# UltronAI/Depth-VO-Feat

Measured on AMD Instinct MI355X. Metric: KITTI 256x832 stereo-seq samples/sec fwd+bwd, higher is better.
Workload: dtype f32

## Files before the change

depth-vo-feat_amd/csrc/conv.hip:

```cpp
#include "dvf_common.h"
#include "conv_op.h"
#include "conv_pipe_host.h"
#include "conv_gather.h"
#include "conv_wgrad.h"
#include "wgrad_pipe.h"

namespace {

__device__ __forceinline__ float act_grad(float g, float yv, int act, float alpha, float beta) {
    if (act == DVF_ACT_RELU) return (yv > 0.f) ? g : 0.f;
    if (act == DVF_ACT_SIGMOID_AFFINE) {
        const float sg = (yv - beta) / alpha;
        return g * alpha * sg * (1.f - sg);
    }
    return g;
}

template <bool VEC>
__global__ __launch_bounds__(256) void act_bwd_kernel(const float *__restrict__ dy, const float *__restrict__ y,
                                                      float *__restrict__ dpre, float *dbias, int C, int HW, int act,
                                                      float alpha, float beta, int chunks, float *part = nullptr, int nper = 0) {
    __shared__ float red[4];
    const int plane = blockIdx.x / chunks, chunk = blockIdx.x - plane * chunks;
    const int c = plane % C;
// ... 558 lines not shown
    return chunks;
}

int64_t dvf_act_bwd_ws_floats(int N, int C, int HW) {
    if (N <= 0 || C <= 0 || HW <= 0) return DVF_ERR_INVALID_ARG;
    const int a = act_bwd_chunks(N, C, HW, true), b = bias_sum_chunks(N, C, HW);
    return (int64_t)C * N * (a > b ? a : b);
}

int dvf_act_bwd(const float *dy, const float *y, float *dpre, float *dbias, int N, int C, int HW, int act, float alpha,
                float beta, int accumulate_dbias, float *ws, int64_t ws_floats, void *stream) {
    if (!dy || (act != DVF_ACT_NONE && !y) || N <= 0 || C <= 0 || HW <= 0) return DVF_ERR_INVALID_ARG;
    if (!dpre && !dbias) return DVF_OK;
    hipStream_t st = dvf_stream(stream);
    if (dbias && !accumulate_dbias && hipMemsetAsync(dbias, 0, sizeof(float) * C, st) != hipSuccess) return DVF_ERR_LAUNCH;
    const bool vec = (HW % 4 == 0) && ((reinterpret_cast<uintptr_t>(dy) | reinterpret_cast<uintptr_t>(y) |
                                        reinterpret_cast<uintptr_t>(dpre)) % 16 == 0);
    const bool sums_only = !dpre && act == DVF_ACT_NONE;
    const int chunks = sums_only ? bias_sum_chunks(N, C, HW) : act_bwd_chunks(N, C, HW, dbias != nullptr);
    const int64_t planes = (int64_t)N * C;
    float *part = (dbias && ws && ws_floats >= dvf_act_bwd_ws_floats(N, C, HW)) ? ws : nullptr;
    if (sums_only) {
        const int per = ((vec ? HW >> 2 : HW) + chunks - 1) / chunks;
        const int threads = per <= 256 ? 64 : per <= 8192 ? 256 : 1024;
        if (vec) bias_sum_kernel<true><<<(unsigned)(planes * chunks), threads, 0, st>>>(dy, dbias, C, HW, chunks, part, N * chunks);
        else bias_sum_kernel<false><<<(unsigned)(planes * chunks), threads, 0, st>>>(dy, dbias, C, HW, chunks, part, N * chunks);
    } else if (vec) act_bwd_kernel<true><<<(unsigned)(planes * chunks), 256, 0, st>>>(dy, y, dpre, dbias, C, HW, act, alpha, beta, chunks, part, N * chunks);
    else act_bwd_kernel<false><<<(unsigned)(planes * chunks), 256, 0, st>>>(dy, y, dpre, dbias, C, HW, act, alpha, beta, chunks, part, N * chunks);
    DVF_LAUNCH_CHECK();
    if (part) {
        bias_finish_kernel<<<C, 64, 0, st>>>(part, dbias, N * chunks);
        DVF_LAUNCH_CHECK();
    }
    return DVF_OK;
}


int64_t dvf_conv2d_packed_floats(const dvf_conv_desc *d, const int *seg_channels, int nseg, int op_kind) {
    return conv_sizes(d, seg_channels, nseg, op_kind, false);
}

int64_t dvf_conv2d_ws_floats(const dvf_conv_desc *d, const int *seg_channels, int nseg, int op_kind) {
    return conv_sizes(d, seg_channels, nseg, op_kind, true);
}

int dvf_conv2d_pack(const dvf_conv_desc *d, const int *seg_channels, int nseg, int op_kind, const float *w, float *packed,
                    void *stream) {
    int rc = check_desc(d);
    if (rc) return rc;
    rc = check_segs(d, seg_channels, nseg);
    if (rc) return rc;
    if (!w || !packed) return DVF_ERR_INVALID_ARG;
    hipStream_t st = dvf_stream(stream);
    if (op_kind == 0) {
        ConvOp op;
        PipePlan pl;
        rc = make_fwd_op(d, seg_channels, nseg, op);
        if (!rc) rc = plan_pipe(op, pl);
        return rc ? rc : launch_pack(op, pl, w, packed, st);
    }
    if (op_kind != 1) return DVF_ERR_INVALID_ARG;
    return for_each_dgrad_seg(d, seg_channels, nseg, true, [&](const DgradSeg &v) -> int {
        return v.packed ? launch_pack(v.op, v.plan, w, packed + v.packed_off, st) : DVF_OK;
    });
}

int dvf_conv2d_fwd(const dvf_conv_desc *d, const float *const *in_segs, const int *seg_channels, int nseg,
                   const float *packed, const float *w, const float *bias, float *out, float *ws, int64_t ws_floats,
                   void *stream) {
    dvf_plan_reset();
    int rc = check_desc(d);
    if (rc) return rc;
    rc = check_segs(d, seg_channels, nseg);
    if (rc) return rc;
    if (!in_segs || !w || !out) return DVF_ERR_INVALID_ARG;
    for (int s = 0; s < nseg; ++s)
        if (!in_segs[s]) return DVF_ERR_INVALID_ARG;
    hipStream_t st = dvf_stream(stream);
    const ConvIO io{in_segs, bias, out, nullptr};
    ConvOp op;
    rc = make_fwd_op(d, seg_channels, nseg, op);
    if (packed && !rc) {
        PipePlan pl;
        rc = plan_pipe(op, pl);
        if (!rc) rc = run_pipe(op, pl, io, packed, ws, ws_floats, st);
        if (rc != DVF_ERR_UNSUPPORTED) return rc;
    }
    return fwd_unpacked(d, op, io, seg_channels, nseg, w, ws, ws_floats, st);
}

int dvf_conv2d_dgrad(const dvf_conv_desc *d, const float *dpre, const float *packed, const float *w, float *const *din_segs,
                     const int *seg_channels, int nseg, float *ws, int64_t ws_floats, const float *const *mask_segs,
                     void *stream) {
    dvf_plan_reset();
    int rc = check_desc(d);
    if (rc) return rc;
    rc = check_segs(d, seg_channels, nseg);
    if (rc) return rc;
    if (!dpre || !w || !din_segs) return DVF_ERR_INVALID_ARG;
    hipStream_t st = dvf_stream(stream);
    auto mask = [&](int s) -> const float * { return mask_segs ? mask_segs[s] : nullptr; };
    if (dvf_head_dgrad_applicable(d, nseg) || (dvf_head_applicable(d, nseg) && !packed))
        return din_segs[0] ? dvf_head_dgrad(d, dpre, w, din_segs[0], st, mask(0)) : DVF_OK;
    return for_each_dgrad_seg(d, seg_channels, nseg, packed != nullptr, [&](const DgradSeg &v) -> int {
        if (!din_segs[v.s]) return DVF_OK;
        const ConvIO io{&dpre, nullptr, din_segs[v.s], mask(v.s)};
        int r = v.packed ? run_pipe(v.op, v.plan, io, packed + v.packed_off, ws, ws_floats, st) : DVF_ERR_UNSUPPORTED;
        if (r == DVF_ERR_UNSUPPORTED) r = dgrad_unpacked(d, v.op, io, w, ws, ws_floats, st);
        return r;
    });
}

int dvf_conv2d_pack_jobs(const dvf_conv_desc *d, const int *seg_channels, int nseg, int op_kind, const float *w, float *packed,
                         void *jobs_host, int max_jobs, int *blocks_out, int *lds_bytes_out) {
    static_assert(sizeof(PackArgs) <= DVF_PACK_JOB_BYTES, "DVF_PACK_JOB_BYTES too small");
    int rc = check_desc(d);
    if (rc) return rc;
    rc = check_segs(d, seg_channels, nseg);
    if (rc) return rc;
    if (!w || !packed || !jobs_host || !blocks_out || max_jobs < 1) return DVF_ERR_INVALID_ARG;
    char *out = static_cast<char *>(jobs_host);
    int njobs = 0;
    auto emit = [&](const ConvOp &op, const PipePlan &pl, float *dst) {
        const PackArgs job = pack_job(op, pl, w, dst, &blocks_out[njobs]);
        memset(out + (size_t)njobs * DVF_PACK_JOB_BYTES, 0, DVF_PACK_JOB_BYTES);
        memcpy(out + (size_t)njobs * DVF_PACK_JOB_BYTES, &job, sizeof(job));
        if (lds_bytes_out && (int)pl.pack_lds > *lds_bytes_out) *lds_bytes_out = (int)pl.pack_lds;
        ++njobs;
    };
    if (op_kind == 0) {
        ConvOp op;
        PipePlan pl;
        rc = make_fwd_op(d, seg_channels, nseg, op);
        if (!rc) rc = plan_pipe(op, pl);
        if (rc) return rc;
        emit(op, pl, packed);
        return njobs;
    }
    if (op_kind != 1) return DVF_ERR_INVALID_ARG;
    rc = for_each_dgrad_seg(d, seg_channels, nseg, true, [&](const DgradSeg &v) -> int {
        if (njobs >= max_jobs) return DVF_ERR_INVALID_ARG;
        if (v.packed) emit(v.op, v.plan, packed + v.packed_off);
        return DVF_OK;
    });
    return rc ? rc : njobs;
}

int dvf_conv2d_pack_batch(const void *jobs_dev, const int *block_prefix_dev, const int *block_job_dev, int njobs,
                          int total_blocks, int lds_bytes, void *stream) {
    if (!jobs_dev || !block_prefix_dev || njobs < 1 || total_blocks < 1 || lds_bytes < 4 || lds_bytes > 64 * 1024)
        return DVF_ERR_INVALID_ARG;
    static_assert(DVF_PACK_JOB_BYTES % alignof(PackArgs) == 0, "job stride");
    static_assert(sizeof(PackArgs) == DVF_PACK_JOB_BYTES, "job stride");
    conv_pack_batch_kernel<<<total_blocks, 256, lds_bytes, dvf_stream(stream)>>>(
        static_cast<const PackArgs *>(jobs_dev), block_prefix_dev, block_job_dev, njobs);
    DVF_LAUNCH_CHECK();
    return DVF_OK;
}

#ifdef DVF_TUNING
int dvf_tuning_read_stamps(unsigned long long *out, int max_blocks) {
    if (!out || !g_stamp_buf) return 0;
    const int nb = g_stamp_blocks < max_blocks ? g_stamp_blocks : max_blocks;
    if (hipDeviceSynchronize() != hipSuccess) return DVF_ERR_LAUNCH;
    if (hipMemcpy(out, g_stamp_buf, (size_t)nb * 64, hipMemcpyDeviceToHost) != hipSuccess) return DVF_ERR_LAUNCH;
    return nb;
}
#endif

}
```

depth-vo-feat_amd/csrc/conv_pipe_host.h:

```cpp
#pragma once
#include <string.h>
#include "dvf_common.h"
#include "conv_pipe.h"
#include "conv_op.h"

namespace {

using dvfp::PClass;
using dvfp::PipeArgs;
using dvfp::PipeGeo;
using dvfp::pipe_geo;
using dvfp::PIPE_MAXNPI;
using dvfp::OUT_FUSED;
using dvfp::OUT_ATOMIC;
using dvfp::OUT_WS;

struct alignas(8) PackArgsBody {
    const float *w;
    float *wp;
    int w_mode;
    int Mtot, Rtot, KK, m_base, M;
    int nseg, segC[DVF_MAX_SEGS];
    int ncls, NCH, CK, MB, VW, TBU;
    int TB[4], TA[4];
    int SL[4];
    unsigned wp_off[4];
    signed char tapmap[4][52];
};
struct PackArgs : PackArgsBody { char pad[DVF_PACK_JOB_BYTES - sizeof(PackArgsBody)]; };

__device__ __forceinline__ void pack_block(const PackArgs &a, int g, int mt, float *S) {
    const int tid = threadIdx.x;
    const int MTW = a.MB >> 5, mb = mt / MTW, mtw = mt - mb * MTW, m0 = mt * 32;
    int seg_start = 0, gg = g, segc = a.segC[0];
    for (int s = 0; s < a.nseg; ++s) {
        const int nchs = (a.segC[s] + a.CK - 1) / a.CK;
        segc = a.segC[s];
        if (gg < nchs) break;
        gg -= nchs;
        seg_start += a.segC[s];
    }
    const int c0 = gg * a.CK, nch = min(a.CK, segc - c0), r0 = seg_start + c0;
    const int mvalid = min(32, a.M - m0);
    const int CKK = a.CK * a.KK;
    const int SR = CKK | 1;
    constexpr int PU = 8;
    if (a.w_mode == 0) {
        const int run = nch * a.KK, total = mvalid * run;
        const float *src = a.w + ((int64_t)(a.m_base + m0) * a.Rtot + r0) * a.KK;
        const int64_t mstride = (int64_t)a.Rtot * a.KK;
        for (int i0 = tid; i0 < total; i0 += 256 * PU) {
            float v[PU];
            int si[PU];
#pragma unroll
            for (int j = 0; j < PU; ++j) {
                const int i = i0 + j * 256;
                if (i < total) {
                    const int m = i / run, x = i - m * run;
                    v[j] = src[m * mstride + x];
                    si[j] = m * SR + x;
                }
            }
#pragma unroll
            for (int j = 0; j < PU; ++j)
                if (i0 + j * 256 < total) S[si[j]] = v[j];
        }
    } else {
        const int run = mvalid * a.KK, total = nch * run;
        const float *src = a.w + ((int64_t)r0 * a.Mtot + a.m_base + m0) * a.KK;
        const int64_t rstride = (int64_t)a.Mtot * a.KK;
        for (int i0 = tid; i0 < total; i0 += 256 * PU) {
            float v[PU];
            int si[PU];
#pragma unroll
            for (int j = 0; j < PU; ++j) {
                const int i = i0 + j * 256;
                if (i < total) {
                    const int rl = i / run, x = i - rl * run, m = x / a.KK, tap = x - m * a.KK;
                    v[j] = src[rl * rstride + x];
                    si[j] = m * SR + rl * a.KK + tap;
                }
            }
#pragma unroll
            for (int j = 0; j < PU; ++j)
                if (i0 + j * 256 < total) S[si[j]] = v[j];
        }
    }
    __syncthreads();
    const int CKH = a.CK >> 1, CPG = CKH / a.VW, LV = 64 * a.VW;
    if (a.VW == 4) {
        typedef float f4 __attribute__((ext_vector_type(4)));
        const int lane = tid & 63, kh = lane >> 5, m = lane & 31;
        for (int c = 0; c < a.ncls; ++c) {
            const int TB = a.TB[c], NKU = a.TA[c] * CPG * a.TBU;
            float *dst = a.wp + a.wp_off[c] + (int64_t)(mb * a.NCH + g) * a.SL[c] + (int64_t)mtw * 256 + lane * 4;
            int ku = tid >> 6, u = ku, cpg = 0, ta = 0;
            while (u >= a.TBU) { u -= a.TBU; if (++cpg == CPG) { cpg = 0; ++ta; } }
            for (; ku < NKU; ku += 4) {
                f4 v = {0.f, 0.f, 0.f, 0.f};
                if (u < TB && m < mvalid) {
                    const float *src = S + m * SR + a.tapmap[c][ta * TB + u];
#pragma unroll
                    for (int j = 0; j < 4; ++j) {
                        const int rl = 2 * (cpg * 4 + j) + kh;
                        if (rl < nch) v[j] = src[rl * a.KK];
                    }
                }
                *reinterpret_cast<f4 *>(dst + (int64_t)ku * MTW * 256) = v;
                u += 4;
                while (u >= a.TBU) { u -= a.TBU; if (++cpg == CPG) { cpg = 0; ++ta; } }
            }
        }
        return;
    }
    const int x = tid & (LV - 1), kstep = 256 / LV;
    const int lane = x / a.VW, j = x - lane * a.VW, kh = lane >> 5, m = lane & 31;
    for (int c = 0; c < a.ncls; ++c) {
        const int TB = a.TB[c], NKU = a.TA[c] * CPG * a.TBU;
        float *dst = a.wp + a.wp_off[c] + (int64_t)(mb * a.NCH + g) * a.SL[c] + (int64_t)mtw * LV + x;
        int ku = tid / LV, u = ku, cpg = 0, ta = 0;
        while (u >= a.TBU) { u -= a.TBU; if (++cpg == CPG) { cpg = 0; ++ta; } }
        for (; ku < NKU; ku += kstep) {
            const int rl = 2 * (cpg * a.VW + j) + kh;
            float v = 0.f;
            if (u < TB && rl < nch && m < mvalid) v = S[m * SR + rl * a.KK + a.tapmap[c][ta * TB + u]];
            dst[(int64_t)ku * MTW * LV] = v;
            u += kstep;
            while (u >= a.TBU) { u -= a.TBU; if (++cpg == CPG) { cpg = 0; ++ta; } }
        }
    }
}

__global__ __launch_bounds__(256) void conv_pack_kernel(const PackArgs a) {
    extern __shared__ float S[];
    pack_block(a, blockIdx.x, blockIdx.y, S);
}

__global__ __launch_bounds__(256) void conv_pack_batch_kernel(const PackArgs *jobs, const int *prefix, const int *block_job,
                                                              int njobs) {
    extern __shared__ float S[];
    const int b = blockIdx.x;
    int lo = 0;
    if (block_job) {
        lo = block_job[b];
    } else {
        int hi = njobs;
        while (hi - lo > 1) {
            const int mid = (lo + hi) >> 1;
            if (prefix[mid] <= b) lo = mid; else hi = mid;
        }
    }
    const PackArgs &a = jobs[lo];
    const int local = b - prefix[lo];
    pack_block(a, local % a.NCH, local / a.NCH, S);
}

__global__ void bias_act_kernel(float *y, const float *bias, int C, int64_t HW, int64_t total, int act, float alpha,
                                float beta) {
    for (int64_t i = (int64_t)blockIdx.x * blockDim.x + threadIdx.x; i < total; i += (int64_t)gridDim.x * blockDim.x) {
        const int c = (int)((i / HW) % C);
        float v = y[i];
        if (bias) v += bias[c];
        y[i] = dvfp::apply_act(v, act, alpha, beta);
    }
}

__global__ void splitk_reduce_kernel(const float *ws, float *out, const float *bias, int KS, int64_t slice, int C, int64_t HW,
                                     int act, float alpha, float beta) {
    for (int64_t i = (int64_t)blockIdx.x * blockDim.x + threadIdx.x; i < slice; i += (int64_t)gridDim.x * blockDim.x) {
        float v = ws[i];
        for (int k = 1; k < KS; ++k) v += ws[i + k * slice];
        if (bias) v += bias[(int)((i / HW) % C)];
        out[i] = dvfp::apply_act(v, act, alpha, beta);
    }
}

__global__ __launch_bounds__(256) void splitk_reduce_mask_kernel(const float *ws, float *out, const float *mask, int KS,
                                                                 int64_t slice, int HW, int chunks) {
    const int plane = blockIdx.x / chunks, chunk = blockIdx.x - plane * chunks;
    const int per = (HW + chunks - 1) / chunks;
    const int lo = chunk * per, hi = min(HW, lo + per);
    const int64_t base = (int64_t)plane * HW;
    for (int e = lo + threadIdx.x; e < hi; e += 256) {
        const int64_t i = base + e;
        float v = ws[i];
        for (int k = 1; k < KS; ++k) v += ws[i + k * slice];
        out[i] = mask[i] > 0.f ? v : 0.f;
    }
}

__global__ __launch_bounds__(256) void splitk_reduce_kpar_kernel(const float *ws, float *out, const float *bias, const float *mask,
                                                                 int KS, int64_t slice, int C, int HW, int act, float alpha,
                                                                 float beta) {
    __shared__ float part[3][64];
    const int lane = threadIdx.x & 63, kq = threadIdx.x >> 6;
    const int k0 = (KS * kq) >> 2, k1 = (KS * (kq + 1)) >> 2;
    const int64_t i0 = (int64_t)blockIdx.x * 64, i = i0 + lane;
    float v = 0.f;
    if (i < slice) {
        const float *p = ws + i + (int64_t)k0 * slice;
#pragma unroll 8
        for (int k = k0; k < k1; ++k, p += slice) v += *p;
    }
    if (kq) part[kq - 1][lane] = v;
    __syncthreads();
    if (kq) return;
    if (i >= slice) return;
    v = ((v + part[0][lane]) + part[1][lane]) + part[2][lane];
    if (mask) {
        out[i] = mask[i] > 0.f ? v : 0.f;
        return;
    }
    if (bias) v += bias[(int)((i / HW) % C)];
    out[i] = dvfp::apply_act(v, act, alpha, beta);
}

inline int out_mode_of(bool covers, int KS, const float *ws, int64_t ws_floats, int64_t plan_ws_floats) {
    if (!covers) return OUT_ATOMIC;
    if (KS <= 1) return OUT_FUSED;
    return (ws && ws_floats >= plan_ws_floats) ? OUT_WS : OUT_ATOMIC;
}

template <class Args>
int prepare_output(Args &a, int mode, float *out, float *ws, hipStream_t st) {
    const int64_t total = (int64_t)a.N * a.M * a.OH * a.OW;
    a.out_mode = mode;
    a.out = out;
    if (mode == OUT_WS) { a.out = ws; a.ws_slice = total; }
    if (mode == OUT_ATOMIC && hipMemsetAsync(out, 0, sizeof(float) * total, st) != hipSuccess) return DVF_ERR_LAUNCH;
    return DVF_OK;
}

template <class Args>
int finish_output(const Args &a, bool kpar, const float *ws, float *out, hipStream_t st) {
    const int64_t HW = (int64_t)a.OH * a.OW, total = (int64_t)a.N * a.M * HW, nb = (total + 255) / 256;
    if (a.out_mode == OUT_WS && kpar) {
        splitk_reduce_kpar_kernel<<<(unsigned)((total + 63) / 64), 256, 0, st>>>(ws, out, a.bias, a.mask, a.KS, total, a.M, (int)HW,
                                                                                a.act, a.alpha, a.beta);
        DVF_LAUNCH_CHECK();
    } else if (a.out_mode == OUT_WS && a.mask) {
        int chunks = 1;
        const int64_t planes = (int64_t)a.N * a.M;
        while (planes * chunks < 1024 && HW / (chunks * 2) >= 256) chunks *= 2;
        splitk_reduce_mask_kernel<<<(unsigned)(planes * chunks), 256, 0, st>>>(ws, out, a.mask, a.KS, total, (int)HW, chunks);
        DVF_LAUNCH_CHECK();
    } else if (a.out_mode == OUT_WS) {
        splitk_reduce_kernel<<<(int)(nb > 4096 ? 4096 : nb), 256, 0, st>>>(ws, out, a.bias, a.KS, total, a.M, HW, a.act,
                                                                          a.alpha, a.beta);
        DVF_LAUNCH_CHECK();
    } else if (a.out_mode == OUT_ATOMIC && (a.bias || a.act != DVF_ACT_NONE)) {
        bias_act_kernel<<<(int)(nb > 2048 ? 2048 : nb), 256, 0, st>>>(out, a.bias, a.M, HW, total, a.act, a.alpha, a.beta);
        DVF_LAUNCH_CHECK();
    }
    if (a.out_mode == OUT_ATOMIC && a.mask)
        return dvf_act_bwd(out, a.mask, out, nullptr, a.N, a.M, (int)HW, DVF_ACT_RELU, 1.f, 0.f, 1, nullptr, 0, st);
    return DVF_OK;
}

#ifdef DVF_TUNING
constexpr size_t STAMP_MAX_BLOCKS = 16384;
unsigned long long *g_stamp_buf = nullptr;
int g_stamp_blocks = 0;
#endif
struct PipePlan {
    PipeArgs a;
    int MT, NT, WM, CKH, TBU, threads;
    size_t lds;
    dim3 grid;
    int64_t packed_floats;
    int64_t ws_floats;
    bool reduce_kpar;
    size_t pack_lds;
};

struct PipeOverride { int on, MT, NT, WM, CK, KS, BN, NST; };
inline PipeOverride pipe_override() {
    PipeOverride o{0, 0, 0, 0, 0, 0, 0, 0};
    if (const char *e = dvf_tune("DVF_PIPE_PLAN"))
        if (sscanf(e, "%d,%d,%d,%d,%d,%d,%d", &o.MT, &o.NT, &o.WM, &o.CK, &o.KS, &o.BN, &o.NST) >= 1) o.on = 1;
    return o;
}

struct PipeTiles { int lsw, lsh, TGX, TGY, TGN, BN; double cov; };
inline PipeTiles pipe_tiles(int OHc, int OWc, int N, int ntile, int BNwant, int IS, int TBmax) {
    PipeTiles best{5, 0, 1, ntile, 1, 1, 1e30};
    for (int lsn = 0; lsn <= 5; ++lsn) {
        const int SN = 1 << lsn;
        for (int lsw = 5 - lsn; lsw >= 0; --lsw) {
            const int lsh = 5 - lsn - lsw, SW = 1 << lsw, SH = 1 << lsh;
            for (int TGN = 1; TGN <= ntile; TGN *= 2) {
                const int BN = SN * TGN;
                if (BN != BNwant) continue;
                for (int TGX = 1; TGX * TGN <= ntile; TGX *= 2) {
                    const int TGY = ntile / (TGX * TGN), BW = TGX * SW, BH = TGY * SH;
                    if ((BW - 1) * IS + TBmax > 160) continue;
                    const double cov = (double)cdiv(OWc, BW) * BW * cdiv(OHc, BH) * BH * cdiv(N, BN) * BN;
                    const double narrow = (SW >= 16 ? 0.0 : (SW == 8 ? 0.12 : 0.3)) + (BW >= 32 ? 0.0 : 0.08);
                    const double cost = cov * (1.0 + narrow + 0.02 * lsh + 0.02 * lsn) + 1e-3 * (BW + BH);
                    if (cost < best.cov) best = PipeTiles{lsw, lsh, TGX, TGY, TGN, BN, cost};
                }
            }
        }
    }
    return best;
}


// ... 74 lines not shown
            d.PSRmax = g.PSR > d.PSRmax ? g.PSR : d.PSRmax;
        }
        auto lds_bytes = [&](int CK) { return ((size_t)d.NST * (slab(CK, TAmax) + (size_t)CK * d.PSRmax) + MB) * 4; };
        int CK = TBU >= 5 ? 8 : 16;
        while (CK > 4 && lds_bytes(CK) > PIPE_LDS_BUDGET) CK >>= 1;
        while (CK > 4 && CK / 2 >= maxc) CK >>= 1;
        if (lds_bytes(CK) > PIPE_LDS_BUDGET) {
            d.NST = 2;
            if (lds_bytes(CK) > PIPE_LDS_BUDGET && PIPE_LDS_BUDGET < 150 * 1024) {
                d.NST = 3;
                if (lds_bytes(CK) > 150 * 1024) d.NST = 2;
                if (lds_bytes(CK) > 150 * 1024) return d;
            }
        }
        if (ov.on && ov.CK) { CK = ov.CK; d.NST = 3; if (lds_bytes(CK) > 150 * 1024) d.NST = 2; }
        if (ov.on && ov.NST) d.NST = ov.NST;
        if ((CK != 4 && CK != 8 && CK != 16) || lds_bytes(CK) > 150 * 1024) return d;
        d.ok = 1; d.CK = CK; d.lds = lds_bytes(CK);
        return d;
    };
    int want_x4 = (a.IW % 4 == 0 && (a.BW * a.IS) % 4 == 0) ? 1 : 0;
    if (const char *e = dvf_tune("DVF_PIPE_X4")) want_x4 = want_x4 && atoi(e) != 0;
    const Depth d1 = depth_for(0), d4 = want_x4 ? depth_for(1) : Depth{0, 0, 3, 0, 0};
    static const bool x4_force = dvf_tune("DVF_PIPE_X4") && atoi(dvf_tune("DVF_PIPE_X4")) == 2;
    const bool use4 = d4.ok && (!d1.ok || x4_force || (d4.CK >= d1.CK && d4.NST >= d1.NST));
    const Depth dd = use4 ? d4 : d1;
    if (!dd.ok) return DVF_ERR_UNSUPPORTED;
    a.x4 = use4 ? 1 : 0;
    a.PSRmax = dd.PSRmax;
    const int CK = dd.CK, NST = dd.NST;
    a.NST = NST;
    a.SLmax = slab(CK, TAmax);
    a.NCH = 0;
    for (int s = 0; s < a.nseg; ++s) a.NCH += cdiv(a.segC[s], CK);
    const int mblocks = cdiv(a.M, MB);
    unsigned off = 0;
    for (int i = 0; i < ncls; ++i) {
        const ClassSpec &c = cls[i];
        const int SL = slab(CK, c.TA);
        a.cls[i] = PClass{c.py, c.px, c.by, c.bx, c.TA, c.TB, c.OHc, c.OWc, SL, c.TA, off};
        const int64_t nf = (int64_t)mblocks * a.NCH * SL;
        if ((int64_t)off + nf >= ((int64_t)1 << 29)) return DVF_ERR_UNSUPPORTED;
        off += (unsigned)nf;
    }
    pl.packed_floats = off;
    int KS = KS0;
    if (ov.on && ov.KS) KS = ov.KS;
    if (KS > a.NCH) KS = a.NCH;
    if (KS < 1) KS = 1;
    if ((int64_t)a.NG * KS * ncls > 65535) return DVF_ERR_UNSUPPORTED;
    a.KS = KS;
    pl.ws_floats = (op.covers && KS > 1) ? (int64_t)KS * a.N * a.M * a.OH * a.OW : 0;
    pl.reduce_kpar = KS >= 8 && (int64_t)a.OH * a.OW < ((int64_t)1 << 30);
    for (int s2 = 0; s2 < a.nseg; ++s2)
        if ((int64_t)a.N * a.segC[s2] * a.IH * a.IW * 4 >= ((int64_t)1 << 31) - 16) return DVF_ERR_UNSUPPORTED;
    pl.MT = MT; pl.NT = NT; pl.WM = WM; pl.CKH = CK / 2; pl.TBU = TBU; pl.lds = dd.lds;
    pl.pack_lds = (size_t)32 * ((CK * op.KK) | 1) * sizeof(float);
    if (pl.pack_lds > 64 * 1024) return DVF_ERR_UNSUPPORTED;
    pl.grid = dim3(a.tilesX * a.tilesY, mblocks, a.NG * KS * ncls);
    {
        const int per_chunk = CK * TAmax * TBmax;
        const int64_t kseq = (int64_t)cdiv(a.NCH, KS) * per_chunk;
        static const int blk_knob = dvf_tune("DVF_PIPE_BLK") ? atoi(dvf_tune("DVF_PIPE_BLK")) : -1;
        static const int blk_terms = dvf_tune("DVF_PIPE_BLKT") ? atoi(dvf_tune("DVF_PIPE_BLKT")) : 0;
        const bool deep = MT == 2 && NT == 1 && WM == 1 && CK >= 8 && TBU >= 2 && TBU <= 4 && kseq >= 512 &&
                          ((int64_t)pl.grid.x * pl.grid.y * pl.grid.z <= 256 || pl.lds > 76 * 1024);
        int every = blk_terms > 0 ? (blk_terms + per_chunk / 2) / per_chunk : 1;
        if (every < 1) every = 1;
        a.blk = blk_knob == 0 ? 0 : blk_knob > 0 ? blk_knob : blk_terms > 0 ? (kseq >= 384 ? every : 0) : (deep ? 1 : 0);
    }
    {
        const int64_t nblocks_total = (int64_t)pl.grid.x * pl.grid.y * pl.grid.z;
        static const bool no4p = dvf_tune("DVF_PIPE_NO4P") != nullptr;
        static const int mt1_4p = dvf_tune("DVF_PIPE_MT1_4P") ? atoi(dvf_tune("DVF_PIPE_MT1_4P")) : 1;
        pl.threads = (!no4p && (pl.lds > 76 * 1024 || nblocks_total <= 256 || (MT == 1 && mt1_4p))) ? dvfp::PIPE_THREADS_4P : dvfp::PIPE_THREADS;
    }
    return DVF_OK;
}

int launch_pipe(const PipeArgs &a, const PipePlan &pl, hipStream_t st) {
    using dvfp::launch_pipe_family;
    if (pl.WM == 2) {
        if (pl.NT != 1) return DVF_ERR_UNSUPPORTED;
        return pl.MT == 2 ? launch_pipe_family<2, 1, 2>(a, pl.CKH, pl.TBU, pl.grid, pl.lds, st, pl.threads)
                          : launch_pipe_family<1, 1, 2>(a, pl.CKH, pl.TBU, pl.grid, pl.lds, st, pl.threads);
    }
    if (pl.WM != 1) return DVF_ERR_UNSUPPORTED;
    if (pl.MT == 2 && pl.NT == 2) return DVF_ERR_UNSUPPORTED;
    if (pl.MT == 2) return launch_pipe_family<2, 1, 1>(a, pl.CKH, pl.TBU, pl.grid, pl.lds, st, pl.threads);
    if (pl.NT == 2) return launch_pipe_family<1, 2, 1>(a, pl.CKH, pl.TBU, pl.grid, pl.lds, st, pl.threads);
    return launch_pipe_family<1, 1, 1>(a, pl.CKH, pl.TBU, pl.grid, pl.lds, st, pl.threads);
}

int run_pipe(const ConvOp &op, const PipePlan &pl, const ConvIO &io, const float *packed, float *ws, int64_t ws_floats,
             hipStream_t st) {
    PipeArgs a = pl.a;
    for (int s = 0; s < a.nseg; ++s) {
        a.in[s] = io.in[s];
        if (a.x4 && (reinterpret_cast<uintptr_t>(a.in[s]) & 15)) return DVF_ERR_UNSUPPORTED;
    }
    a.wp = packed; a.bias = io.bias; a.mask = io.mask;
    const int mode = out_mode_of(op.covers, a.KS, ws, ws_floats, pl.ws_floats);
    int rc = prepare_output(a, mode, io.out, ws, st);
    if (rc) return rc;
    if (const char *e = dvf_tune("DVF_DBG")) a.dbg = atoi(e);
    a.stamps = nullptr;
#ifdef DVF_TUNING
    if (dvf_tune("DVF_STAMPS")) {
        const size_t nb = (size_t)pl.grid.x * pl.grid.y * pl.grid.z;
        if (!g_stamp_buf && hipMalloc(&g_stamp_buf, STAMP_MAX_BLOCKS * 64) != hipSuccess) return DVF_ERR_LAUNCH;
        if (nb <= STAMP_MAX_BLOCKS) {
            if (hipMemsetAsync(g_stamp_buf, 0, nb * 64, st) != hipSuccess) return DVF_ERR_LAUNCH;
            a.stamps = g_stamp_buf;
            g_stamp_blocks = (int)nb;
        }
    }
#endif
    dvf_plan_note(DVF_K_PIPE, pl.MT, pl.NT, pl.WM, 2 * pl.CKH, pl.TBU, a.KS, a.BN, a.NST, pl.threads, (int)pl.lds, mode | (a.ncls << 4) | (a.x4 << 8) | ((a.blk ? 1 : 0) << 9));
    if (dvf_tune("DVF_PIPE_DEBUG"))
        fprintf(stderr, "[pipe] M %d chunks %d N %d out %dx%d cls %d | MT %d NT %d WM %d CK %d TBU %d KS %d BN %d tile %dx%d "
                "(sub %dx%d) grid %ux%ux%u lds %zu x%d mode %d\n", a.M, a.NCH, a.N, a.OH, a.OW, a.ncls, pl.MT, pl.NT, pl.WM,
                2 * pl.CKH, pl.TBU, a.KS, a.BN, a.BH, a.BW, 1 << a.lsh, 1 << a.lsw, pl.grid.x, pl.grid.y, pl.grid.z, pl.lds, a.NST, mode);
    rc = launch_pipe(a, pl, st);
    return rc ? rc : finish_output(a, pl.reduce_kpar, ws, io.out, st);
}

PackArgs pack_job(const ConvOp &op, const PipePlan &pl, const float *w, float *packed, int *blocks) {
    const PipeArgs &a = pl.a;
    PackArgs p{};
    p.w = w; p.wp = packed; p.w_mode = op.w_mode; p.Mtot = op.Mtot; p.Rtot = op.Rtot; p.KK = op.KK;
    p.m_base = op.m_base; p.M = a.M; p.nseg = a.nseg;
    for (int s = 0; s < a.nseg; ++s) p.segC[s] = a.segC[s];
    p.ncls = op.ncls; p.NCH = a.NCH; p.CK = 2 * pl.CKH; p.MB = 32 * pl.MT * pl.WM; p.VW = pl.CKH >= 4 ? 4 : pl.CKH;
    p.TBU = pl.TBU;
    for (int c = 0; c < op.ncls; ++c) {
        p.SL[c] = a.cls[c].SL;
        p.TB[c] = op.cls[c].TB;
        p.TA[c] = op.cls[c].TA;
        p.wp_off[c] = a.cls[c].wp_off;
        for (int t = 0; t < op.cls[c].TA * op.cls[c].TB; ++t) p.tapmap[c][t] = (signed char)op.cls[c].tapmap[t];
    }
    *blocks = a.NCH * cdiv(a.M, p.MB) * (p.MB >> 5);
    return p;
}

int launch_pack(const ConvOp &op, const PipePlan &pl, const float *w, float *packed, hipStream_t st) {
    int blocks;
    const PackArgs p = pack_job(op, pl, w, packed, &blocks);
    conv_pack_kernel<<<dim3(p.NCH, blocks / p.NCH), 256, pl.pack_lds, st>>>(p);
    DVF_LAUNCH_CHECK();
    return DVF_OK;
}

}
```

depth-vo-feat_amd/dvf/conv.py:

```python
import ctypes
import math
import weakref

import torch
import torch.nn as nn

from . import lib as L


def _c(t):
    return t if (t.dtype == torch.float32 and t.is_contiguous()) else t.float().contiguous()


class _NullCtx:
    def __enter__(self):
        return self

    def __exit__(self, *exc):
        return False


_NULL = _NullCtx()


def conv_out_size(h, k, stride, pad, opad, transposed):
    return (h - 1) * stride - 2 * pad + k + opad if transposed else (h + 2 * pad - k) // stride + 1


_WS = {}


def _workspace(nfloats, device, raw_stream=None, stream=None):
    capturing = torch.cuda.is_current_stream_capturing()
    key = (device, L.stream_raw() if raw_stream is None else raw_stream)
    buf = None if capturing else _WS.get(key)
    if buf is None or buf.numel() < nfloats:
        with (torch.cuda.stream(stream) if stream is not None else _NULL):
            if capturing:
                return torch.empty(max(int(nfloats), 1), device=device, dtype=torch.float32)
            _WS[key] = buf = torch.empty(max(int(nfloats), 1 << 20), device=device, dtype=torch.float32)
    return buf


_PACK_REGISTRY = []
_PACK_TABLES = {}
_PACK_SMALL_LDS = 20 * 1024


def _stamp(w):
    return (w.data_ptr(), w._version, getattr(w, "_dvf_epoch", 0), L.PACK_EPOCH)


def repack_all(owner=None, bucket=None):
    if not _PACK_REGISTRY:
        return
    lib = L.lib()
    live = [(r, r[0]()) for r in _PACK_REGISTRY]
    live = [(r, w) for r, w in live if w is not None]
    if len(live) != len(_PACK_REGISTRY) and not torch.cuda.is_current_stream_capturing():
        _PACK_REGISTRY[:] = [r for r, _ in live]
    if owner is not None:
        live = [(r, w) for r, w in live if getattr(w, "_dvf_owner", None) is owner and w._dvf_bucket == bucket]
    if not live:
        return
    t = _PACK_TABLES.setdefault((id(owner) if owner is not None else 0, bucket), {"n": -1})
    key = tuple((id(r), w.data_ptr()) for r, w in live)
    if t.get("key") != key:
        if torch.cuda.is_current_stream_capturing():
            for r, w in live:
                _, desc, segc, kind, ent = r
                L.check(lib.dvf_conv2d_pack(ctypes.byref(desc), L.int_array(segc), len(segc), kind, L.dev(w), L.dev(ent[0]),
                                            L.stream()), "dvf_conv2d_pack")
                ent[1] = _stamp(w)
            return
        groups = {}
        for r, w in live:
            _, desc, segc, kind, ent = r
            buf = (ctypes.c_char * (L.PACK_JOB_BYTES * len(segc)))()
            nb = (ctypes.c_int * len(segc))()
            lds = ctypes.c_int(4)
            n = lib.dvf_conv2d_pack_jobs(ctypes.byref(desc), L.int_array(segc), len(segc), kind, L.dev(w), L.dev(ent[0]),
                                         ctypes.cast(buf, ctypes.c_void_p), len(segc), nb, ctypes.byref(lds))
            if n < 0:
                L.check(n, "dvf_conv2d_pack_jobs")
            g = groups.setdefault(0 if lds.value <= _PACK_SMALL_LDS else 1, {"blobs": [], "blocks": [], "lds": 4})
            g["blobs"].append(bytes(buf)[: n * L.PACK_JOB_BYTES])
            g["blocks"] += list(nb[:n])
            g["lds"] = max(g["lds"], lds.value)
        dev = live[0][1].device
        t.setdefault("keep", []).append(t.get("launches"))
        t["launches"] = []
        for _, g in sorted(groups.items()):
            blocks = g["blocks"]
            prefix = [0]
            for b in blocks:
                prefix.append(prefix[-1] + b)
            t["launches"].append({
                "jobs": torch.frombuffer(bytearray(b"".join(g["blobs"])), dtype=torch.uint8).to(dev),
                "prefix": torch.tensor(prefix, dtype=torch.int32, device=dev),
                "block_job": torch.repeat_interleave(torch.arange(len(blocks), dtype=torch.int32),
                                                     torch.tensor(blocks, dtype=torch.int64)).to(dev),
                "njobs": len(blocks), "total": prefix[-1], "lds": g["lds"]})
        t["key"] = key
    for q in t["launches"]:
        L.check(lib.dvf_conv2d_pack_batch(q["jobs"].data_ptr(), q["prefix"].data_ptr(), q["block_job"].data_ptr(), q["njobs"],
                                          q["total"], q["lds"], L.stream()), "dvf_conv2d_pack_batch")
    for r, w in live:
        r[4][1] = _stamp(w)


def _packed_weights(weight, holder, desc, segc, kind, pkey=None, segarr=None):
    cache = holder.__dict__.get("_dvf_pack")
    if cache is None:
        cache = holder.__dict__["_dvf_pack"] = {}
    if pkey is None:
        pkey = (desc.N, desc.H_in, desc.W_in, desc.H_out, desc.W_out, desc.stride, desc.pad, desc.transposed, tuple(segc))
    key = (kind, pkey)
    ent = cache.get(key)
    if ent is None:
        lib = L.lib()
        if segarr is None:
            segarr = L.int_array(segc)
        nf = lib.dvf_conv2d_packed_floats(ctypes.byref(desc), segarr, len(segc), kind)
        wsf = max(int(lib.dvf_conv2d_ws_floats(ctypes.byref(desc), segarr, len(segc), kind)), 0)
        if nf == L.ERR_UNSUPPORTED:
            cache[key] = ent = [None, None, wsf]
        else:
            if nf < 0:
                L.check(int(nf), "dvf_conv2d_packed_floats")
            cache[key] = ent = [torch.zeros(int(nf), device=weight.device, dtype=torch.float32), None, wsf]
            _PACK_REGISTRY.append([weakref.ref(holder), desc, list(segc), kind, ent])
    buf = ent[0]
    if buf is None:
        return None, (_workspace(ent[2], weight.device) if ent[2] else None)
    stamp = (holder.data_ptr(), holder._version, getattr(holder, "_dvf_epoch", 0), L.PACK_EPOCH)
    if ent[1] != stamp:
        with L.timed("conv_pack", 0.0, 8.0 * weight.numel()):
            L.check(L.lib().dvf_conv2d_pack(ctypes.byref(desc), L.int_array(segc), len(segc), kind, L.dev(weight, "weight"),
                                            L.dev(buf), L.stream()), "dvf_conv2d_pack")
        ent[1] = stamp
    return buf, (_workspace(ent[2], weight.device) if ent[2] else None)


DETERMINISTIC = False


def set_deterministic(on=True):
    global DETERMINISTIC
    DETERMINISTIC = bool(on)


def _bias_sums(lib, dy, y, dpre, dbias, N, C, HW, act, alpha, beta, accumulate):
    ws = _workspace(int(lib.dvf_act_bwd_ws_floats(N, C, HW)), dy.device) if (DETERMINISTIC and dbias is not None) else None
    L.check(lib.dvf_act_bwd(L.dev(dy, "grad_out"), L.dev(y), L.dev(dpre), L.dev(dbias), N, C, HW, act, alpha, beta,
                            1 if accumulate else 0, L.dev(ws), ws.numel() if ws is not None else 0, L.stream()), "dvf_act_bwd")


def _wgrad_ws_floats(holder, desc, segc):
    cache = holder.__dict__.setdefault("_dvf_wgws", {})
    key = (desc.N, desc.H_in, desc.W_in, desc.H_out, desc.W_out, desc.stride, desc.pad, desc.transposed, tuple(segc))
    n = cache.get(key)
    if n is None:
        n = int(L.lib().dvf_conv2d_wgrad_ws_floats(ctypes.byref(desc), L.int_array(segc), len(segc)))
        cache[key] = n = max(n, 0)
    return n


GEOM_LOG = None
FUSE_RELU_BWD = True


class ReluTag:
    __slots__ = ()


class _Geo:
    __slots__ = ("desc", "dref", "segc", "segarr", "nseg", "cin0", "cout", "oh", "ow", "macs", "tag", "pkey")

    def __init__(self, weight, cfg, inputs):
        k, stride, pad, opad, transposed, act, alpha, beta, out_hw = cfg[:9]
        N, _, H, W = inputs[0].shape
        self.segc = segc = [int(x.shape[1]) for x in inputs]
        self.nseg, self.cin0 = len(segc), segc[0]
        self.segarr = L.int_array(segc)
        cin = sum(segc)
        self.cout = cout = weight.shape[1] if transposed else weight.shape[0]
        if (weight.shape[0] if transposed else weight.shape[1]) != cin:
            raise ValueError(f"weight {tuple(weight.shape)} does not match {cin} input channels")
        oh, ow = conv_out_size(H, k, stride, pad, opad, transposed), conv_out_size(W, k, stride, pad, opad, transposed)
        if out_hw is not None:
            oh, ow = min(oh, out_hw[0]), min(ow, out_hw[1])
        self.oh, self.ow = oh, ow
        self.desc = L.ConvDesc(N, cin, H, W, cout, oh, ow, k, k, stride, pad, 1 if transposed else 0, act, alpha, beta)
        self.dref = ctypes.byref(self.desc)
        taps = k * k / (stride * stride) if transposed else k * k
        self.macs = float(N) * cout * oh * ow * cin * taps
        self.tag = f"{'T' if transposed else 'C'}{k}x{k}s{stride} {cin}->{cout} in{H}x{W} out{oh}x{ow} N{N}"
        self.pkey = (N, H, W, oh, ow, stride, pad, 1 if transposed else 0, tuple(segc))


class ConvFn(torch.autograd.Function):

    @staticmethod
    def forward(ctx, weight, bias, cfg, *inputs):
        k, stride, pad, opad, transposed, act, alpha, beta, out_hw = cfg[:9]
        ctx.out_tag = cfg[9] if len(cfg) > 9 else None
        ctx.in_tags = [getattr(x, "_dvf_relu_tag", None) for x in inputs]
        ctx.wparam = weight if getattr(weight, "_dvf_grad", None) is not None else None
        ctx.bparam = bias if (bias is not None and getattr(bias, "_dvf_grad", None) is not None) else None
        ctx.holder = weight
        inputs = [_c(x) for x in inputs]
        weight = _c(weight)
        bias = _c(bias) if bias is not None else None
        x0 = inputs[0]
        N, _, H, W = x0.shape
        gkey = (cfg[:9], N, H, W) if len(inputs) == 1 else (cfg[:9], N, H, W) + tuple(x.shape[1] for x in inputs[1:])
        geos = ctx.holder.__dict__.get("_dvf_geo")
        if geos is None:
            geos = ctx.holder.__dict__["_dvf_geo"] = {}
        g = geos.get(gkey)
        if g is None:
            g = geos[gkey] = _Geo(weight, cfg, inputs)
        elif g.cin0 != x0.shape[1]:
            raise ValueError(f"weight {tuple(weight.shape)} does not match {sum(int(x.shape[1]) for x in inputs)} input channels")
        if g.nseg > 1:
            for x in inputs:
                if x.shape[0] != N or x.shape[2] != H or x.shape[3] != W:
                    raise ValueError(f"virtual concat needs equal N,H,W; got {[tuple(t.shape) for t in inputs]}")
        desc, segc, cout, oh, ow = g.desc, g.segc, g.cout, g.oh, g.ow
# ... 292 lines not shown
```

Before: 650.6.

## Make weight-pack batch kernel persistent with register prefetch of next unit

Replaces the one-block-per-unit weight pack batch kernel with a persistent grid sized to a few blocks per CU. Each block loops over units, loading the next unit's weights into registers (vectorized when aligned) while it stores the current tile from LDS. The change also merges small and large LDS jobs into one launch group by raising the small-LDS threshold. It adds templated register-count variants and more register pressure, and it may reduce parallelism when units are few.

Result: no change. 653.9 (median of 4 runs) (+0.5%).

```diff
diff --git a/depth-vo-feat_amd/csrc/conv.hip b/depth-vo-feat_amd/csrc/conv.hip
--- a/depth-vo-feat_amd/csrc/conv.hip
+++ b/depth-vo-feat_amd/csrc/conv.hip
@@ -734,10 +734,33 @@
         return DVF_ERR_INVALID_ARG;
     static_assert(DVF_PACK_JOB_BYTES % alignof(PackArgs) == 0, "job stride");
     static_assert(sizeof(PackArgs) == DVF_PACK_JOB_BYTES, "job stride");
-    conv_pack_batch_kernel<<<total_blocks, 256, lds_bytes, dvf_stream(stream)>>>(
-        static_cast<const PackArgs *>(jobs_dev), block_prefix_dev, block_job_dev, njobs);
-    DVF_LAUNCH_CHECK();
-    return DVF_OK;
+    static_assert(sizeof(PackArgsBody::tapmap) == PACK_TAPMAP_WORDS * 4, "tap map words");
+    static const int cus = [] {
+        int dev = 0, n = 0;
+        if (hipGetDevice(&dev) != hipSuccess ||
+            hipDeviceGetAttribute(&n, hipDeviceAttributeMultiprocessorCount, dev) != hipSuccess || n < 1) n = 256;
+        return n;
+    }();
+    int bpc = PACK_BPC, nstage = PACK_NSTAGE, prefetch = 1;
+    if (const char *e = dvf_tune("DVF_PACK_BPC")) bpc = atoi(e);
+    if (const char *e = dvf_tune("DVF_PACK_NSTAGE")) nstage = atoi(e);
+    if (const char *e = dvf_tune("DVF_PACK_PREFETCH")) prefetch = atoi(e) != 0;
+    if (nstage != 1) nstage = 2;
+    const int tile_floats = (lds_bytes + 3) / 4, stage_floats = tile_floats + PACK_TAPMAP_WORDS;
+    const int fit = (int)(PACK_CU_LDS / ((size_t)nstage * stage_floats * sizeof(float) + 512));
+    if (bpc > fit) bpc = fit;
+    if (bpc < 1) bpc = 1;
+    const int64_t want = (int64_t)bpc * cus;
+    const int grid = (int)(want < total_blocks ? want : total_blocks);
+    const PackArgs *jobs = static_cast<const PackArgs *>(jobs_dev);
+    hipStream_t st = dvf_stream(stream);
+    if (tile_floats <= 12 * 256)
+        return launch_pack_batch<12>(jobs, block_prefix_dev, block_job_dev, njobs, total_blocks, stage_floats, nstage, prefetch, grid, st);
+    if (tile_floats <= 20 * 256)
+        return launch_pack_batch<20>(jobs, block_prefix_dev, block_job_dev, njobs, total_blocks, stage_floats, nstage, prefetch, grid, st);
+    if (tile_floats <= 28 * 256)
+        return launch_pack_batch<28>(jobs, block_prefix_dev, block_job_dev, njobs, total_blocks, stage_floats, nstage, prefetch, grid, st);
+    return launch_pack_batch<64>(jobs, block_prefix_dev, block_job_dev, njobs, total_blocks, stage_floats, nstage, prefetch, grid, st);
 }
 
 #ifdef DVF_TUNING
diff --git a/depth-vo-feat_amd/csrc/conv_pipe_host.h b/depth-vo-feat_amd/csrc/conv_pipe_host.h
--- a/depth-vo-feat_amd/csrc/conv_pipe_host.h
+++ b/depth-vo-feat_amd/csrc/conv_pipe_host.h
@@ -136,23 +136,241 @@
     pack_block(a, blockIdx.x, blockIdx.y, S);
 }
 
-__global__ __launch_bounds__(256) void conv_pack_batch_kernel(const PackArgs *jobs, const int *prefix, const int *block_job,
-                                                              int njobs) {
-    extern __shared__ float S[];
-    const int b = blockIdx.x;
+struct PackUnit {
+    const PackArgs *a;
+    int g, mt, nch, mvalid;
+    const float *src;
+    int64_t stride;
+    int vec;
+    int runv, total;
+    int dq, dr;
+};
+
+__device__ __forceinline__ void pack_chunk(const PackArgs &a, int g, int &r0, int &nch) {
+    int seg_start = 0, gg = g, segc = a.segC[0];
+#pragma unroll
+    for (int s = 0; s < DVF_MAX_SEGS; ++s) {
+        if (s >= a.nseg) break;
+        const int nchs = (a.segC[s] + a.CK - 1) / a.CK;
+        segc = a.segC[s];
+        if (gg < nchs) break;
+        gg -= nchs;
+        seg_start += a.segC[s];
+    }
+    const int c0 = gg * a.CK;
+    nch = min(a.CK, segc - c0);
+    r0 = seg_start + c0;
+}
+
+__device__ __forceinline__ PackUnit pack_unit(const PackArgs *__restrict__ jobs, const int *__restrict__ prefix,
+                                              const int *__restrict__ unit_job, int njobs, int u) {
     int lo = 0;
-    if (block_job) {
-        lo = block_job[b];
+    if (unit_job) {
+        lo = unit_job[u];
     } else {
         int hi = njobs;
         while (hi - lo > 1) {
             const int mid = (lo + hi) >> 1;
-            if (prefix[mid] <= b) lo = mid; else hi = mid;
+            if (prefix[mid] <= u) lo = mid; else hi = mid;
         }
     }
     const PackArgs &a = jobs[lo];
-    const int local = b - prefix[lo];
-    pack_block(a, local % a.NCH, local / a.NCH, S);
+    const int local = u - prefix[lo];
+    PackUnit q;
+    q.a = &a;
+    q.g = local % a.NCH;
+    q.mt = local / a.NCH;
+    int r0;
+    pack_chunk(a, q.g, r0, q.nch);
+    const int m0 = q.mt * 32;
+    q.mvalid = min(32, a.M - m0);
+    int64_t base;
+    int rows, run;
+    if (a.w_mode == 0) {
+        rows = q.mvalid; run = q.nch * a.KK; q.stride = (int64_t)a.Rtot * a.KK;
+        base = ((int64_t)(a.m_base + m0) * a.Rtot + r0) * a.KK;
+    } else {
+        rows = q.nch; run = q.mvalid * a.KK; q.stride = (int64_t)a.Mtot * a.KK;
+        base = ((int64_t)r0 * a.Mtot + a.m_base + m0) * a.KK;
+    }
+    q.src = a.w + base;
+    q.vec = (((uintptr_t)q.src | (uintptr_t)(q.stride * 4)) & 15) == 0 && (run & 3) == 0;
+    q.runv = q.vec ? run >> 2 : run;
+    q.total = rows * q.runv;
+    q.dq = 256 / q.runv;
+    q.dr = 256 - q.dq * q.runv;
+    return q;
+}
+
+template <int NR>
+__device__ __forceinline__ void pack_fetch(const PackUnit &q, float (&v)[NR], int &tm, int &row0, int &x0) {
+    typedef float f4 __attribute__((ext_vector_type(4)));
+    typedef const float __attribute__((address_space(1))) *gsrc_t;
+    typedef const f4 __attribute__((address_space(1))) *gsrc4_t;
+    const gsrc_t src = (gsrc_t)q.src;
+    const int tid = threadIdx.x;
+    tm = tid < 52 ? reinterpret_cast<const int *>(&q.a->tapmap[0][0])[tid] : 0;
+    const int runv = q.runv, total = q.total, dq = q.dq, dr = q.dr;
+    int row = tid / runv, x = tid - row * runv;
+    row0 = row; x0 = x;
+    if (q.vec) {
+#pragma unroll
+        for (int j = 0; j < NR / 4; ++j) {
+            const int64_t off = tid + j * 256 < total ? row * q.stride + 4 * x : 0;
+            const f4 t = *(gsrc4_t)(src + off);
+            v[4 * j] = t[0]; v[4 * j + 1] = t[1]; v[4 * j + 2] = t[2]; v[4 * j + 3] = t[3];
+            x += dr;
+            const int wrap = x >= runv;
+            x -= wrap ? runv : 0;
+            row += dq + wrap;
+        }
+    } else {
+#pragma unroll
+        for (int j = 0; j < NR; ++j) {
+            const int64_t off = tid + j * 256 < total ? row * q.stride + x : 0;
+            v[j] = src[off];
+            x += dr;
+            const int wrap = x >= runv;
+            x -= wrap ? runv : 0;
+            row += dq + wrap;
+        }
+    }
+}
+
+template <int NR>
+__device__ __forceinline__ void pack_commit(const PackUnit &q, const float (&v)[NR], int tm, int row, int x, float *S, int *T) {
+    const PackArgs &a = *q.a;
+    const int tid = threadIdx.x;
+    if (tid < 52) T[tid] = tm;
+    const int SR = (a.CK * a.KK) | 1, KK = a.KK;
+    const int runv = q.runv, total = q.total, dq = q.dq, dr = q.dr;
+    const unsigned inv = ((1u << 20) + KK - 1) / KK;
+    if (q.vec) {
+#pragma unroll
+        for (int j = 0; j < NR / 4; ++j) {
+            if (tid + j * 256 < total) {
+#pragma unroll
+                for (int e = 0; e < 4; ++e) {
+                    const int xe = 4 * x + e;
+                    int si = row * SR + xe;
+                    if (a.w_mode) si = xe + row * KK + (int)(((unsigned)xe * inv) >> 20) * (SR - KK);
+                    S[si] = v[4 * j + e];
+                }
+            }
+            x += dr;
+            const int wrap = x >= runv;
+            x -= wrap ? runv : 0;
+            row += dq + wrap;
+        }
+    } else {
+#pragma unroll
+        for (int j = 0; j < NR; ++j) {
+            if (tid + j * 256 < total) {
+                int si = row * SR + x;
+                if (a.w_mode) si = x + row * KK + (int)(((unsigned)x * inv) >> 20) * (SR - KK);
+                S[si] = v[j];
+            }
+            x += dr;
+            const int wrap = x >= runv;
+            x -= wrap ? runv : 0;
+            row += dq + wrap;
+        }
+    }
+}
+
+__device__ __forceinline__ void pack_store(const PackUnit &q, const float *S, const int *T) {
+    const PackArgs &a = *q.a;
+    const signed char *tapmap = reinterpret_cast<const signed char *>(T);
+    typedef float __attribute__((address_space(1))) *gdst_t;
+    const gdst_t wp = (gdst_t)a.wp;
+    const int tid = threadIdx.x, g = q.g, nch = q.nch, mvalid = q.mvalid;
+    const int MTW = a.MB >> 5, mb = q.mt / MTW, mtw = q.mt - mb * MTW;
+    const int SR = (a.CK * a.KK) | 1;
+    const int CKH = a.CK >> 1, CPG = CKH / a.VW, LV = 64 * a.VW;
+    if (a.VW == 4) {
+        typedef float f4 __attribute__((ext_vector_type(4)));
+        typedef f4 __attribute__((address_space(1))) *gdst4_t;
+        const int lane = tid & 63, kh = lane >> 5, m = lane & 31;
+        for (int c = 0; c < a.ncls; ++c) {
+            const int TB = a.TB[c], NKU = a.TA[c] * CPG * a.TBU;
+            const gdst_t dst = wp + a.wp_off[c] + (int64_t)(mb * a.NCH + g) * a.SL[c] + (int64_t)mtw * 256 + lane * 4;
+            int ku = tid >> 6, u = ku, cpg = 0, ta = 0;
+            while (u >= a.TBU) { u -= a.TBU; if (++cpg == CPG) { cpg = 0; ++ta; } }
+            for (; ku < NKU; ku += 4) {
+                f4 v = {0.f, 0.f, 0.f, 0.f};
+                if (u < TB && m < mvalid) {
+                    const float *src = S + m * SR + tapmap[c * 52 + ta * TB + u];
+#pragma unroll
+                    for (int j = 0; j < 4; ++j) {
+                        const int rl = 2 * (cpg * 4 + j) + kh;
+                        if (rl < nch) v[j] = src[rl * a.KK];
+                    }
+                }
+                *(gdst4_t)(dst + (int64_t)ku * MTW * 256) = v;
+                u += 4;
+                while (u >= a.TBU) { u -= a.TBU; if (++cpg == CPG) { cpg = 0; ++ta; } }
+            }
+        }
+    } else {
+        const int x = tid & (LV - 1), kstep = 256 / LV;
+        const int lane = x / a.VW, j = x - lane * a.VW, kh = lane >> 5, m = lane & 31;
+        for (int c = 0; c < a.ncls; ++c) {
+            const int TB = a.TB[c], NKU = a.TA[c] * CPG * a.TBU;
+            const gdst_t dst = wp + a.wp_off[c] + (int64_t)(mb * a.NCH + g) * a.SL[c] + (int64_t)mtw * LV + x;
+            int ku = tid / LV, u = ku, cpg = 0, ta = 0;
+            while (u >= a.TBU) { u -= a.TBU; if (++cpg == CPG) { cpg = 0; ++ta; } }
+            for (; ku < NKU; ku += kstep) {
+                const int rl = 2 * (cpg * a.VW + j) + kh;
+                float v = 0.f;
+                if (u < TB && rl < nch && m < mvalid) v = S[m * SR + rl * a.KK + tapmap[c * 52 + ta * TB + u]];
+                dst[(int64_t)ku * MTW * LV] = v;
+                u += kstep;
+                while (u >= a.TBU) { u -= a.TBU; if (++cpg == CPG) { cpg = 0; ++ta; } }
+            }
+        }
+    }
+}
+
+constexpr int PACK_TAPMAP_WORDS = 52;
+constexpr int PACK_BPC = 6;
+constexpr int PACK_NSTAGE = 1;
+constexpr size_t PACK_CU_LDS = 160 * 1024;
+
+template <int NR>
+__global__ __launch_bounds__(256) void conv_pack_batch_kernel(const PackArgs *__restrict__ jobs, const int *__restrict__ prefix,
+                                                              const int *__restrict__ unit_job, int njobs, int units,
+                                                              int stage_floats, int nstage, int prefetch) {
+    extern __shared__ float S[];
+    float v[NR];
+    int tm;
+#ifndef DVF_TUNING
+    prefetch = 1;
+#endif
+    int u = blockIdx.x;
+    if (u >= units) return;
+    int row0, x0;
+    PackUnit q = pack_unit(jobs, prefix, unit_job, njobs, u);
+    pack_fetch<NR>(q, v, tm, row0, x0);
+    for (int stage = 0;; stage ^= nstage - 1) {
+        float *Ss = S + stage * stage_floats;
+        int *Ts = reinterpret_cast<int *>(Ss + stage_floats - PACK_TAPMAP_WORDS);
+        pack_commit<NR>(q, v, tm, row0, x0, Ss, Ts);
+        __syncthreads();
+        u += gridDim.x;
+        const bool more = u < units;
+        PackUnit nxt = q;
+        if (more) {
+            nxt = pack_unit(jobs, prefix, unit_job, njobs, u);
+            if (prefetch) pack_fetch<NR>(nxt, v, tm, row0, x0);
+        }
+        pack_store(q, Ss, Ts);
+        if (!more) break;
+        if (nstage == 1) __syncthreads();
+#ifdef DVF_TUNING
+        if (!prefetch) pack_fetch<NR>(nxt, v, tm, row0, x0);
+#endif
+        q = nxt;
+    }
 }
 
 __global__ void bias_act_kernel(float *y, const float *bias, int C, int64_t HW, int64_t total, int act, float alpha,
@@ -533,4 +751,22 @@
     return DVF_OK;
 }
 
-}
+template <int NR>
+int launch_pack_batch(const PackArgs *jobs, const int *prefix, const int *unit_job, int njobs, int units, int stage_floats,
+                             int nstage, int prefetch, int grid, hipStream_t st) {
+    const size_t lds = (size_t)nstage * stage_floats * sizeof(float);
+    if (lds > 64 * 1024) {
+        static bool raised = false;
+        if (!raised) {
+            if (hipFuncSetAttribute(reinterpret_cast<const void *>(&conv_pack_batch_kernel<NR>),
+                                    hipFuncAttributeMaxDynamicSharedMemorySize, 2 * 65 * 1024) != hipSuccess)
+                return DVF_ERR_LAUNCH;
+            raised = true;
+        }
+    }
+    conv_pack_batch_kernel<NR><<<grid, 256, lds, st>>>(jobs, prefix, unit_job, njobs, units, stage_floats, nstage, prefetch);
+    DVF_LAUNCH_CHECK();
+    return DVF_OK;
+}
+
+}
diff --git a/depth-vo-feat_amd/dvf/conv.py b/depth-vo-feat_amd/dvf/conv.py
--- a/depth-vo-feat_amd/dvf/conv.py
+++ b/depth-vo-feat_amd/dvf/conv.py
@@ -44,7 +44,8 @@
 
 _PACK_REGISTRY = []
 _PACK_TABLES = {}
-_PACK_SMALL_LDS = 20 * 1024
+_PACK_SMALL_LDS = 64 * 1024
+_PACK_PAIR_JOBS = False
 
 
 def _stamp(w):
@@ -74,7 +75,8 @@
                 ent[1] = _stamp(w)
             return
         groups = {}
-        for r, w in live:
+        order = sorted(live, key=lambda rw: (rw[1].data_ptr(), rw[0][3])) if _PACK_PAIR_JOBS else live
+        for r, w in order:
             _, desc, segc, kind, ent = r
             buf = (ctypes.c_char * (L.PACK_JOB_BYTES * len(segc)))()
             nb = (ctypes.c_int * len(segc))()
```
